# ucla-rlcourse/competitive-rl

Hardware: NVIDIA B200
Metric: cPongDouble env-steps/sec at 84x84x4 obs (higher is better)
Workload: dtype u8 obs / int32+f64 game state / f32 area-resize

## Files before the change

### competitive-rl_b200/csrc/crl_abi.cu

```cuda
#include <math.h>
#include <stdarg.h>
#include <stdio.h>
#include <stdlib.h>
#include <string.h>

#include <cuda.h>

#include <atomic>
#include <mutex>
#include <unordered_map>
#include <vector>

#include "../../include/crl_b200.h"
#include "crl_host.h"
#include "pong_common.cuh"

using namespace crl;

static thread_local char g_err[512] = "";
static std::atomic<uint64_t> g_launches{0};

static int fail(int code, const char* fmt, ...) {
    va_list ap;
    va_start(ap, fmt);
// ... 1 lines not shown
    va_end(ap);
    return code;
}

int crl_set_error(int code, const char* fmt, ...) {
    va_list ap;
    va_start(ap, fmt);
    vsnprintf(g_err, sizeof g_err, fmt, ap);
    va_end(ap);
    return code;
}
void crl_count_launch(int n) { g_launches += (uint64_t)n; }

#define CUDA_TRY(expr)                                                                                \
    do {                                                                                              \
        cudaError_t _e = (expr);                                                                      \
        if (_e != cudaSuccess) return fail(CRL_E_CUDA, "%s: %s", #expr, cudaGetErrorString(_e));      \
    } while (0)

#define LAUNCH(expr)     \
    do {                 \
        CUDA_TRY(expr);  \
        g_launches += 1; \
    } while (0)

struct crl_pong {
    crl_pong_config cfg;
    PongDev dev;
    std::vector<void*> allocs;
    double* serves_dev = nullptr;
    uint8_t* atlas_dev = nullptr;
    uint8_t* text_tab_dev = nullptr;
    uint8_t* tmpl_dev = nullptr;
    AreaTabs* tabs_dev = nullptr;
    AreaTabs tabs_host;
    uint8_t* fast_tabs_dev = nullptr;
    int32_t* actions_stage = nullptr;
    float* rew_stage = nullptr;
    uint8_t* done_stage = nullptr;
    int32_t* steps_stage = nullptr;
    float* real_stage = nullptr;
    bool atlas_loaded = false;
    bool was_reset = false;
    cudaStream_t copy_stream = nullptr;
    cudaEvent_t ev_state = nullptr, ev_copied = nullptr;
    struct ObsSet {
        uint8_t* obs[2];
        FrameSpec* shown;
        bool valid;
    };
    std::vector<ObsSet> sets;
    FrameSpec* shown_dev = nullptr;
    bool full_obs = false;
};

static size_t obs_bytes(const crl_pong* h) {
    return (size_t)h->dev.n * (h->dev.ring ? 2 * h->dev.c : h->dev.c) * h->dev.dim * h->dev.dim;
}

static void obs_written(crl_pong* h, const void* p, size_t bytes) {
    if (!p) return;
    const uintptr_t a = (uintptr_t)p, b = a + bytes, ob = obs_bytes(h);
    for (auto& st : h->sets)
        for (int k = 0; k < h->dev.n_agents; ++k)
            if (a < (uintptr_t)st.obs[k] + ob && (uintptr_t)st.obs[k] < b) st.valid = false;
}

static bool build_axis(int ssize, int dsize, uint8_t* src0, uint8_t* cnt, float (*alpha)[MAX_TAPS], uint8_t* first,
                       uint8_t* last) {
    const double scale = (double)ssize / dsize;
    for (int s = 0; s < ssize; ++s) { first[s] = 255; last[s] = 0; }
    for (int dx = 0; dx < dsize; ++dx) {
        const double fsx1 = dx * scale, fsx2 = fsx1 + scale;
        const double cell = fmin(scale, ssize - fsx1);
        int sx1 = (int)ceil(fsx1), sx2 = (int)floor(fsx2);
        sx2 = sx2 < ssize - 1 ? sx2 : ssize - 1;
        sx1 = sx1 < sx2 ? sx1 : sx2;
        int n = 0, s0 = -1;
        auto emit = [&](int s, float a) -> bool {
            if (n == 0) s0 = s;
            if (n >= MAX_TAPS || s != s0 + n) return false;
            alpha[dx][n++] = a;
            if (first[s] == 255) first[s] = (uint8_t)dx;
            last[s] = (uint8_t)dx;
            return true;
        };
        if (sx1 - fsx1 > 1e-3 && !emit(sx1 - 1, (float)((sx1 - fsx1) / cell))) return false;
        for (int sx = sx1; sx < sx2; ++sx)
            if (!emit(sx, (float)(1.0 / cell))) return false;
        if (fsx2 - sx2 > 1e-3 && !emit(sx2, (float)(fmin(fmin(fsx2 - sx2, 1.0), cell) / cell))) return false;
        if (n == 0) return false;
        src0[dx] = (uint8_t)s0;
        cnt[dx] = (uint8_t)n;
        for (int k = n; k < MAX_TAPS; ++k) alpha[dx][k] = 0.f;
    }
    for (int s = 0; s < ssize; ++s)
        if (first[s] == 255) return false;
    return true;
}

static bool build_tabs(int dim, AreaTabs* t) {
    memset(t, 0, sizeof *t);
    t->dim = dim;
    if (!build_axis(SCREEN_W, dim, t->x_src0, t->x_n, t->x_a, t->x_first, t->x_last)) return false;
    if (!build_axis(SCREEN_H, dim, t->y_src0, t->y_n, t->y_b, t->y_first, t->y_last)) return false;
    for (int dx = 0; dx < dim; ++dx)
// ... 62 lines not shown
    h->cfg = *cfg;
    PongDev& d = h->dev;
    memset(&d, 0, sizeof d);
    const size_t n = (size_t)cfg->num_envs;
    d.n = cfg->num_envs;
    d.n_agents = cfg->n_agents;
    d.dim = cfg->resized_dim;
    d.c = cfg->frame_stack > 0 ? cfg->frame_stack : 1;
    d.max_rounds = cfg->max_num_rounds;
    d.ring = cfg->stack_mode == 1 ? 1 : 0;
    d.zero_on_done = cfg->zero_on_done ? 1 : 0;
    d.first_env = cfg->first_env;
    d.seed = cfg->seed;
    const int dd = d.dim * d.dim;
    d.text_stride = ((tabs.text_rows * d.dim + 15) / 16) * 16;
    if (d.text_stride > ((dd + 15) / 16) * 16) d.text_stride = ((dd + 15) / 16) * 16;
    d.text_w0 = 0; d.text_w1 = d.text_stride / 4;
#define ALLOC(ptr, count)                                                        \
    do {                                                                         \
        cudaError_t _e = dev_alloc(h, &(ptr), (count));                          \
        if (_e != cudaSuccess) {                                                 \
            crl_pong_destroy(h);                                                 \
            return fail(CRL_E_CUDA, "cudaMalloc: %s", cudaGetErrorString(_e));   \
        }                                                                        \
    } while (0)
    ALLOC(d.ball, n); ALLOC(d.vx, n); ALLOC(d.vy, n); ALLOC(d.bats, n); ALLOC(d.score, n);
    ALLOC(d.num_steps, n); ALLOC(d.clip_steps, n); ALLOC(d.serve_count, n); ALLOC(d.last_done, n);
    ALLOC(d.skipbuf, 2 * n); ALLOC(d.hist, d.c * n); ALLOC(d.term_hist, d.c * n);
    ALLOC(d.serve_overrun, 1);
    ALLOC(d.stats, 8);
    ALLOC(d.work_counter, 2);
    ALLOC(h->tabs_dev, 1);
    ALLOC(h->atlas_dev, (size_t)CRL_PONG_ATLAS_BYTES);
    ALLOC(h->text_tab_dev, (size_t)ATLAS_SCORES * ATLAS_SCORES * 3 * 2 * d.text_stride);
    ALLOC(h->tmpl_dev, (size_t)((dd + 15) / 16) * 16);
    ALLOC(h->actions_stage, 2 * n); ALLOC(h->rew_stage, 2 * n); ALLOC(h->done_stage, n);
    ALLOC(h->steps_stage, n); ALLOC(h->real_stage, 2 * n);
    h->tabs_host = tabs;
    const size_t ftb = pong_fast_tabs_bytes(d.dim);
    if (ftb) {
        std::vector<uint8_t> img(ftb);
        if (pong_fast_tabs_fill(tabs, d.text_stride, img.data())) {
            ALLOC(h->fast_tabs_dev, ftb);
            cudaError_t _e = cudaMemcpy(h->fast_tabs_dev, img.data(), ftb, cudaMemcpyHostToDevice);
            if (_e == cudaSuccess) _e = launch_pong_build_bat_lut(d.dim, h->fast_tabs_dev, 0);
            if (_e != cudaSuccess) {
                crl_pong_destroy(h);
                return fail(CRL_E_CUDA, "fast tabs upload: %s", cudaGetErrorString(_e));
            }
            g_launches += 1;
            d.fast_tabs = h->fast_tabs_dev;
            d.quad_ok = (pong_quad_ok(tabs) && getenv("CRL_PONG_NO_QUAD") == nullptr) ? 1 : 0;
            h->full_obs = getenv("CRL_PONG_FULL_OBS") != nullptr;
        }
    }
    d.tabs = h->tabs_dev;
    d.atlas = h->atlas_dev;
    d.text_tab = h->text_tab_dev;
    d.tmpl = h->tmpl_dev;
#undef ALLOC
    e = cudaMemcpy(h->tabs_dev, &tabs, sizeof tabs, cudaMemcpyHostToDevice);
    if (e == cudaSuccess) e = pong_raster_init(d.raster_grid);
    if (e == cudaSuccess) e = launch_pong_construct(d, 0);
    if (e == cudaSuccess) e = cudaDeviceSynchronize();
    if (e != cudaSuccess) {
        crl_pong_destroy(h);
        return fail(CRL_E_CUDA, "construct: %s", cudaGetErrorString(e));
    }
    g_launches += 1;
    *out = h;
    return CRL_OK;
}

#define CHECK_HANDLE(h)                                        \
    do {                                                       \
        if (!(h)) return fail(CRL_E_INVALID, "null handle");   \
    } while (0);                                               \
    CrlDeviceGuard crl_guard_((h)->cfg.device);                \
    CUDA_TRY(crl_guard_.err)

int crl_pong_load_atlas(crl_pong* h, const uint8_t* strips_host, size_t bytes, void* stream) {
    CHECK_HANDLE(h);
    if (!strips_host || bytes != (size_t)CRL_PONG_ATLAS_BYTES)
        return fail(CRL_E_INVALID, "atlas must be %d bytes ([22][22][34][160][3] uint8)", CRL_PONG_ATLAS_BYTES);
    cudaStream_t s = (cudaStream_t)stream;
    {
        const AreaTabs& t = h->tabs_host;
        const int first = t.y_src0[t.text_rows - 1];
        bool white = true;
        for (int pair = 0; pair < ATLAS_SCORES * ATLAS_SCORES && white; ++pair)
            for (int r = first; r < ATLAS_ROWS && white; ++r) {
                const uint8_t* row = strips_host + ((size_t)pair * ATLAS_ROWS + r) * SCREEN_W * 3;
                for (int i = 0; i < SCREEN_W * 3; ++i)
                    if (row[i] != 255) { white = false; break; }
            }
        h->dev.fast_ok = white ? 1 : 0;
    }
    CUDA_TRY(cudaMemcpyAsync(h->atlas_dev, strips_host, bytes, cudaMemcpyHostToDevice, s));
    LAUNCH(launch_pong_build_tables(h->dev, h->text_tab_dev, h->tmpl_dev, s));
    CUDA_TRY(cudaStreamSynchronize(s));
    {
        const int tw = h->dev.text_stride / 4;
        const size_t n_ent = (size_t)ATLAS_SCORES * ATLAS_SCORES * 3 * 2;
        std::vector<uint32_t> tt(n_ent * tw), tm(tw);
        CUDA_TRY(cudaMemcpy(tt.data(), h->text_tab_dev, tt.size() * sizeof(uint32_t), cudaMemcpyDeviceToHost));
        CUDA_TRY(cudaMemcpy(tm.data(), h->tmpl_dev, tm.size() * sizeof(uint32_t), cudaMemcpyDeviceToHost));
        int w0 = tw, w1 = 0;
        for (int w = 0; w < tw; ++w) {
            bool differs = tm[w] != tt[w];
            for (size_t e = 1; e < n_ent && !differs; ++e) differs = tt[e * tw + w] != tt[w];
            if (differs) { if (w < w0) w0 = w; w1 = w + 1; }
        }
        if (w1 <= w0) w0 = w1 = 0;
        if (getenv("CRL_PONG_TEXT_FULL") != nullptr) { w0 = 0; w1 = tw; }
        h->dev.text_w0 = w0; h->dev.text_w1 = w1;
    }
    h->atlas_loaded = true;
    for (auto& st : h->sets) st.valid = false;
    return CRL_OK;
}

int crl_pong_inject_serves(crl_pong* h, const double* serves_host, int32_t k, void* stream) {
    CHECK_HANDLE(h);
    if (!serves_host || k < 3) return fail(CRL_E_INVALID, "serve table needs k >= 3 entries per env");
    cudaStream_t s = (cudaStream_t)stream;
    double* buf = nullptr;
    CUDA_TRY(dev_alloc(h, &buf, (size_t)h->dev.n * k * 2));
    CUDA_TRY(cudaMemcpyAsync(buf, serves_host, (size_t)h->dev.n * k * 2 * sizeof(double), cudaMemcpyHostToDevice, s));
    h->serves_dev = buf;
    h->dev.serves = buf;
    h->dev.serves_k = k;
    LAUNCH(launch_pong_construct(h->dev, s));
    CUDA_TRY(cudaStreamSynchronize(s));
    h->was_reset = false;
    return CRL_OK;
}

int crl_pong_seed(crl_pong* h, uint64_t seed) {
    CHECK_HANDLE(h);
    h->dev.seed = seed;
    return CRL_OK;
}

static int need_ready(crl_pong* h, bool need_reset) {
    if (!h->atlas_loaded) return fail(CRL_E_STATE, "crl_pong_load_atlas must be called before reset/step");
    if (need_reset && !h->was_reset) return fail(CRL_E_STATE, "reset must be called before step");
    return CRL_OK;
}

int crl_pong_render_obs(crl_pong* h, uint8_t* obs0_dev, uint8_t* obs1_dev, void* stream) {
    CHECK_HANDLE(h);
    if (int r = need_ready(h, true)) return r;
// ... 1 lines not shown
    if (h->dev.n_agents == 1) obs1_dev = obs0_dev;
    cudaStream_t s = (cudaStream_t)stream;
    crl_pong::ObsSet* set = nullptr;
    for (auto& st : h->sets)
        if (st.obs[0] == obs0_dev && (h->dev.n_agents == 1 || st.obs[1] == obs1_dev)) set = &st;
    const bool incremental = !h->full_obs && pong_raster_incremental_ok(h->dev, obs0_dev, obs1_dev);
    if (set && set->valid && incremental) {
        LAUNCH(launch_pong_raster(h->dev, h->dev.hist, obs0_dev, obs1_dev, set->shown, s));
        return CRL_OK;
    }
    LAUNCH(launch_pong_raster(h->dev, h->dev.hist, obs0_dev, obs1_dev, nullptr, s));
    if (!set) {
        obs_written(h, obs0_dev, obs_bytes(h));
        obs_written(h, obs1_dev, obs_bytes(h));
    } else if (incremental) {
        const size_t per_agent = (size_t)h->dev.c * h->dev.n;
        for (int k = 0; k < h->dev.n_agents; ++k)
            CUDA_TRY(cudaMemcpyAsync(set->shown + k * per_agent, h->dev.hist, per_agent * sizeof(FrameSpec),
                                     cudaMemcpyDeviceToDevice, s));
        set->valid = true;
    } else {
        set->valid = false;
    }
    return CRL_OK;
}

int crl_pong_set_obs_buffers(crl_pong* h, uint8_t* const* obs0_devs_host, uint8_t* const* obs1_devs_host, int32_t count,
                             void* stream) {
    CHECK_HANDLE(h);
    const int na = h->dev.n_agents;
    if (count != 0) {
        if (h->dev.ring) return fail(CRL_E_STATE, "stack_mode ring keeps its own frames: there are no buffer sets to register");
        if (count < 0 || count > CRL_PONG_MAX_OBS_SETS || !obs0_devs_host || (na == 2 && !obs1_devs_host))
            return fail(CRL_E_INVALID, "need 1 .. %d buffer sets (and obs1 buffers for cPongDouble), got %d",
                        CRL_PONG_MAX_OBS_SETS, count);
        std::vector<uint8_t*> all;
        for (int i = 0; i < count; ++i)
            for (int k = 0; k < na; ++k) {
                uint8_t* b = k ? obs1_devs_host[i] : obs0_devs_host[i];
                if (!b) return fail(CRL_E_INVALID, "null buffer in set %d", i);
                for (uint8_t* o : all)
                    if (o == b) return fail(CRL_E_INVALID, "a buffer appears twice in the sets");
                all.push_back(b);
            }
    }
    CUDA_TRY(cudaStreamSynchronize((cudaStream_t)stream));
    h->sets.clear();
    if (h->shown_dev) {
        CUDA_TRY(cudaFree(h->shown_dev));
        h->shown_dev = nullptr;
    }
    if (count == 0) return CRL_OK;
    const size_t per_set = (size_t)na * h->dev.c * h->dev.n;
    CUDA_TRY(cudaMalloc(&h->shown_dev, (size_t)count * per_set * sizeof(FrameSpec)));
    for (int i = 0; i < count; ++i)
        h->sets.push_back({{obs0_devs_host[i], na == 2 ? obs1_devs_host[i] : obs0_devs_host[i]}, h->shown_dev + i * per_set, false});
    return CRL_OK;
}

int crl_pong_forget_obs(crl_pong* h) {
    if (!h) return fail(CRL_E_INVALID, "null handle");
    for (auto& st : h->sets) st.valid = false;
    return CRL_OK;
}

int crl_pong_render_obs_generic(crl_pong* h, uint8_t* obs0_dev, uint8_t* obs1_dev, void* stream) {
    CHECK_HANDLE(h);
    if (int r = need_ready(h, true)) return r;
    if (!obs0_dev || (h->dev.n_agents == 2 && !obs1_dev)) return fail(CRL_E_INVALID, "null observation buffer");
    LAUNCH(launch_pong_raster_generic(h->dev, h->dev.hist, nullptr, h->dev.ring, obs0_dev, obs1_dev, (cudaStream_t)stream));
    obs_written(h, obs0_dev, obs_bytes(h));
    obs_written(h, obs1_dev, obs_bytes(h));
    return CRL_OK;
}

int crl_pong_render_obs_f32(crl_pong* h, int32_t terminal, const uint8_t* only_done_dev, float* obs0_dev, float* obs1_dev, void* stream) {
    CHECK_HANDLE(h);
    if (int r = need_ready(h, true)) return r;
    if (h->dev.ring) return fail(CRL_E_STATE, "float32 observations are plain stacks: create the handle with stack_mode 0");
    if (!obs0_dev || (h->dev.n_agents == 2 && !obs1_dev)) return fail(CRL_E_INVALID, "null observation buffer");
    LAUNCH(launch_pong_raster_f32(h->dev, terminal ? h->dev.term_hist : h->dev.hist, only_done_dev, obs0_dev, obs1_dev, (cudaStream_t)stream));
    obs_written(h, obs0_dev, 4 * obs_bytes(h));
    obs_written(h, obs1_dev, 4 * obs_bytes(h));
    return CRL_OK;
}

int crl_pong_reset_state(crl_pong* h, void* stream) {
    CHECK_HANDLE(h);
    if (int r = need_ready(h, false)) return r;
    LAUNCH(launch_pong_reset(h->dev, (cudaStream_t)stream));
    h->was_reset = true;
    h->dev.ring_phase = 0;
    h->dev.fill_all = 1;
    return CRL_OK;
}

int crl_pong_reset(crl_pong* h, uint8_t* obs0_dev, uint8_t* obs1_dev, void* stream) {
    CHECK_HANDLE(h);
    if (int r = need_ready(h, false)) return r;
    LAUNCH(launch_pong_reset(h->dev, (cudaStream_t)stream));
    h->was_reset = true;
    h->dev.ring_phase = 0;
    h->dev.fill_all = 1;
    return crl_pong_render_obs(h, obs0_dev, obs1_dev, stream);
}

// ... 255 lines not shown
```

### competitive-rl_b200/csrc/pong_common.cuh

```cuda
#pragma once
#include <cuda_runtime.h>
#include <stdint.h>

namespace crl {

constexpr int SCREEN_W = 160;
constexpr int SCREEN_H = 210;
constexpr int ARENA_TOP = 34;
constexpr int ARENA_BOTTOM = 194;
constexpr int ARENA_CENTERY = 114;
constexpr int BALL_SIZE = 4;
constexpr int BALL_X0 = 78;
constexpr int BALL_Y0 = 112;
constexpr int BAT_W = 5;
constexpr int BAT_H = 15;
constexpr int BAT_Y0 = 107;
constexpr int LEFT_BAT_X = 16;
constexpr int RIGHT_BAT_X = 139;
constexpr int SPEED = 4;
constexpr int MAX_STEP_PER_ROUND = 10000;
constexpr int CHEAT_CODES = 999;
constexpr int MIRROR_ROW = 25;
constexpr int ATLAS_ROWS = 34;
constexpr int ATLAS_SCORES = 22;
// ... 13 lines not shown
}

struct AreaTabs {
    int dim;
    int text_rows;
    uint8_t x_src0[MAX_DIM], x_n[MAX_DIM];
    uint8_t y_src0[MAX_DIM], y_n[MAX_DIM];
    float x_a[MAX_DIM][MAX_TAPS];
    float x_pa[MAX_DIM][MAX_TAPS];
    float y_b[MAX_DIM][MAX_TAPS];
    uint8_t x_first[SCREEN_W], x_last[SCREEN_W];
    uint8_t y_first[SCREEN_H], y_last[SCREEN_H];
};

struct PongDev {
    int n;
    int n_agents;
    int dim;
    int c;
    int max_rounds;
    int ring;
    int ring_phase;
    int fill_all;
    int zero_on_done;
    int64_t first_env;
    uint64_t seed;
    int32_t* ball;
    double* vx;
    double* vy;
    int32_t* bats;
    int32_t* score;
    int32_t* num_steps;
    int32_t* clip_steps;
    int32_t* serve_count;
    uint8_t* last_done;
    RenderState* skipbuf;
    FrameSpec* hist;
    FrameSpec* term_hist;
    const double* serves;
    int serves_k;
    int32_t* serve_overrun;
    unsigned long long* stats;
    unsigned long long* work_counter;
    const AreaTabs* tabs;
    const uint8_t* atlas;
    const uint8_t* text_tab;
    const uint8_t* tmpl;
    int text_stride;
    int text_w0, text_w1;
    const void* fast_tabs;
    int fast_ok;
    int raster_grid[3];
    int quad_ok;
};

__host__ __device__ inline void philox4x32_10(uint32_t c0, uint32_t c1, uint32_t c2, uint32_t c3, uint32_t k0,
                                              uint32_t k1, uint32_t out[4]) {
    for (int r = 0; r < 10; ++r) {
        uint64_t p0 = (uint64_t)0xD2511F53u * c0;
        uint64_t p1 = (uint64_t)0xCD9E8D57u * c2;
        uint32_t n0 = (uint32_t)(p1 >> 32) ^ c1 ^ k0;
        uint32_t n1 = (uint32_t)p1;
        uint32_t n2 = (uint32_t)(p0 >> 32) ^ c3 ^ k1;
        uint32_t n3 = (uint32_t)p0;
        c0 = n0; c1 = n1; c2 = n2; c3 = n3;
        k0 += 0x9E3779B9u;
        k1 += 0xBB67AE85u;
    }
    out[0] = c0; out[1] = c1; out[2] = c2; out[3] = c3;
}

cudaError_t launch_pong_construct(const PongDev& p, cudaStream_t s);
cudaError_t launch_pong_reset(const PongDev& p, cudaStream_t s);
cudaError_t launch_pong_step(const PongDev& p, const int32_t* actions, float* rew, uint8_t* done, int32_t* num_steps,
                             float* real_reward, cudaStream_t s);
cudaError_t launch_pong_get_state(const PongDev& p, double* state, cudaStream_t s);
cudaError_t launch_pong_set_state(const PongDev& p, const double* state, cudaStream_t s);
cudaError_t launch_pong_random_actions(int32_t* actions, int n_values, uint64_t seed, uint64_t step, cudaStream_t s);

cudaError_t launch_pong_build_tables(const PongDev& p, uint8_t* text_tab, uint8_t* tmpl, cudaStream_t s);
cudaError_t launch_pong_raster(const PongDev& p, const FrameSpec* hist, uint8_t* obs0, uint8_t* obs1, FrameSpec* shown,
                               cudaStream_t s);
bool pong_raster_incremental_ok(const PongDev& p, const void* obs0, const void* obs1);
cudaError_t launch_pong_raster_generic(const PongDev& p, const FrameSpec* hist, const uint8_t* only_done, int ring,
                                       uint8_t* obs0, uint8_t* obs1, cudaStream_t s);
cudaError_t launch_pong_raster_f32(const PongDev& p, const FrameSpec* hist, const uint8_t* only_done, float* obs0, float* obs1,
                                   cudaStream_t s);
cudaError_t pong_raster_init(int grid_out[3]);
bool pong_quad_ok(const AreaTabs& a);
size_t pong_fast_tabs_bytes(int dim);
bool pong_fast_tabs_fill(const AreaTabs& a, int text_stride, void* host_buf);
cudaError_t launch_pong_build_bat_lut(int dim, void* fast_tabs_dev, cudaStream_t s);
cudaError_t launch_pong_raw_frame(const PongDev& p, int env, uint8_t* rgb0, uint8_t* rgb1, cudaStream_t s);

}
```

### competitive-rl_b200/csrc/pong_raster_fast.cu

```cuda
#include <type_traits>

#include "pong_raster_dev.cuh"

namespace crl {

template <int TAPS> struct alignas(16) TapEnt;
template <> struct alignas(16) TapEnt<3> { uint32_t meta; float w[3]; };
template <> struct alignas(16) TapEnt<5> { uint32_t meta; float w[5]; uint32_t pad[2]; };

#ifndef CRL_FAST84_CTAS
#define CRL_FAST84_CTAS 3
#endif
template <int DIM> struct FastCfg;
template <> struct FastCfg<84> { static constexpr int TAPS = 3, VEC = 16, CTAS = CRL_FAST84_CTAS; };
template <> struct FastCfg<42> { static constexpr int TAPS = 5, VEC = 4, CTAS = 3; };

constexpr int FAST_WARPS = 8;
constexpr int FIRST_PAD = 224;
constexpr int BAT_ROWS = 8;

template <int DIM> struct alignas(16) FastTabs {
    TapEnt<FastCfg<DIM>::TAPS> xe[DIM], ye[DIM];
    uint32_t bat_lut[2][DIM][1 << FastCfg<DIM>::TAPS];
    float xlut[DIM][1 << FastCfg<DIM>::TAPS];
// ... 133 lines not shown
    any_valid = va || vb;
    if (!va) f.y = f.w;
    if (!vb) f.w = f.y;
    const int pairA = (int)(f.y & 255u) * ATLAS_SCORES + (int)((f.y >> 8) & 255u);
    const int pairB = (int)(f.w & 255u) * ATLAS_SCORES + (int)((f.w >> 8) & 255u);
    int base = pairA, kind = 0;
    if (pairA != pairB) {
        const int d = pairB - pairA;
        if (d == ATLAS_SCORES) kind = 1;
        else if (d == 1 && (pairA % ATLAS_SCORES) != ATLAS_SCORES - 1) kind = 2;
        else if (d == -ATLAS_SCORES) { base = pairB; kind = 1; }
        else if (d == -1 && (pairB % ATLAS_SCORES) != ATLAS_SCORES - 1) { base = pairB; kind = 2; }
        else return -2;
    }
    return (base * 3 + kind) * 2 + agent;
}

template <int DIM>
__device__ __forceinline__ void frame_patch_offsets(const FastTabs<DIM>* T, FrameSpec f, int agent, int lane, int& bat_off,
                                                    int& ball_off) {
    const int cL = (int)T->bat_c0[0], cR = (int)T->bat_c0[1];
    const int b_side = lane >> 4, b_which = (lane >> 3) & 1, b_row = lane & 7;
    const int p_which = lane >> 4, p_col = lane & 3, p_row = (lane >> 2) & 3;
    if (!((f.y >> 16) & 1u)) { f.x = f.z; f.y = f.w; }
    if (!((f.w >> 16) & 1u)) { f.z = f.x; f.w = f.y; }
    const bool same = (f.x == f.z);
    const int lyA = (f.x >> 16) & 255u, ryA = f.x >> 24, lyB = (f.z >> 16) & 255u, ryB = f.z >> 24;
    const int vlA = agent ? ryA : lyA, vrA = agent ? lyA : ryA;
    const int vlB = agent ? ryB : lyB, vrB = agent ? lyB : ryB;
    bat_off = -1;
    {
        const int y0 = b_which ? (b_side ? vrB : vlB) : (b_side ? vrA : vlA);
        const int c0 = max(y0, ARENA_TOP), c1 = min(y0 + BAT_H, ARENA_BOTTOM);
        if (c1 > c0 && !(b_which && same)) {
            const int dy = (int)T->y_first[c0] + b_row;
            if (dy <= (int)T->y_last[c1 - 1]) bat_off = dy * DIM + (b_side ? cR : cL);
        }
    }
    ball_off = -1;
    {
        const FrameSpec& g = f;
        const uint32_t bx = p_which ? g.z : g.x;
        int x0 = bx & 255u, x1 = min(x0 + BALL_SIZE, SCREEN_W);
        int y0 = (bx >> 8) & 255u, y1 = min(y0 + BALL_SIZE, ARENA_BOTTOM);
        y0 = max(y0, ARENA_TOP);
        if (agent) { const int t = SCREEN_W - x1; x1 = SCREEN_W - x0; x0 = t; }
        if (x1 > x0 && y1 > y0 && !(p_which && same)) {
            const int dx = (int)T->x_first[x0] + p_col, dy = (int)T->y_first[y0] + p_row;
            if (dx <= (int)T->x_last[x1 - 1] && dy <= (int)T->y_last[y1 - 1]) ball_off = dy * DIM + dx;
        }
    }
}

template <int DIM, bool RING, bool INC>
__global__ void __launch_bounds__(FAST_WARPS * 32, FastCfg<DIM>::CTAS)
pong_raster_fast_kernel(PongDev p, const FrameSpec* __restrict__ hist, uint8_t* __restrict__ obs0,
                        uint8_t* __restrict__ obs1, const FastTabs<DIM>* __restrict__ gtabs, FrameSpec* __restrict__ shown) {
    constexpr int TAPS = FastCfg<DIM>::TAPS, VEC = FastCfg<DIM>::VEC;
    constexpr int DD = DIM * DIM, FB = ((DD + 15) / 16) * 16, NCH = DD / VEC;
#ifndef CRL_RASTER_TMA
#define CRL_RASTER_TMA 0
#endif
    constexpr bool USE_TMA = (DD % 16 == 0) && (CRL_RASTER_TMA != 0) && !INC;
    constexpr int TEXT_ITERS = 3;
    typedef typename VecT<VEC>::type V;
    typedef FastTabs<DIM> Tabs;
    static_assert(DD % VEC == 0, "frame must be a whole number of store vectors");
    static_assert(!INC || (!RING && VEC == 16), "incremental stacks: 16-byte chunks, plain stacks");

    extern __shared__ uint4 smem_raw[];
    uint8_t* smem = reinterpret_cast<uint8_t*>(smem_raw);
    const Tabs* T = reinterpret_cast<const Tabs*>(smem);
    const int lane = threadIdx.x & 31, warp = threadIdx.x >> 5;
    uint8_t* sm8 = smem + sizeof(Tabs) + (size_t)warp * FB;
    V* sm = reinterpret_cast<V*>(sm8);

    {
        const uint4* src = reinterpret_cast<const uint4*>(gtabs);
        uint4* dst = reinterpret_cast<uint4*>(smem);
        for (int i = threadIdx.x; i < (int)(sizeof(Tabs) / 16); i += blockDim.x) dst[i] = src[i];
        const uint4* tm = reinterpret_cast<const uint4*>(p.tmpl);
        uint4* f = reinterpret_cast<uint4*>(sm8);
        for (int i = lane; i < FB / 16; i += 32) f[i] = tm[i];
    }
    __syncthreads();

    const int text_chunks = p.text_stride / VEC;
    const int cL = (int)T->bat_c0[0], cR = (int)T->bat_c0[1];
    const int b_side = lane >> 4, b_which = (lane >> 3) & 1, b_row = lane & 7;
    const int p_which = lane >> 4, p_col = lane & 3, p_row = (lane >> 2) & 3;
    int prev_bat_off = -1, prev_ball_off = -1;
    uint32_t prev_bat_rest = 0u, prev_ball_old = 0u;
    int cur_text = -1;
    bool pending = false;
    FrameSpec prev_spec = make_uint4(0u, 0u, 0u, 0u);
    bool prev_known = false;

    const long long n_stacks = (long long)p.n * p.n_agents;
    const int per_ticket = INC ? CRL_INC_TICKET : max(1, 4 / (RING ? 2 : p.c));
    const int out_slots = RING ? 2 * p.c : p.c;
    long long s = 0, s_end = 0;
    for (;;) {
        if (s >= s_end) {
            unsigned long long ticket = 0ull;
            if (lane == 0) ticket = atomicAdd(p.work_counter, (unsigned long long)per_ticket);
            s = (long long)__shfl_sync(0xffffffffu, ticket, 0);
            s_end = min(s + per_ticket, n_stacks);
            if (s >= n_stacks) break;
        }
        const long long s_cur = s++;
        const int env = (int)(s_cur / p.n_agents), agent = (int)(s_cur % p.n_agents);
        uint8_t* out_stack = (agent ? obs1 : obs0) + (size_t)env * out_slots * DD;
        FrameSpec my_spec = make_uint4(0u, 0u, 0u, 0u), my_shown = make_uint4(0u, 0u, 0u, 0u);
        FrameSpec* shown_at = INC ? shown + ((size_t)agent * p.c + lane) * p.n + env : nullptr;
        if (lane < p.c) {
            my_spec = hist[(size_t)lane * p.n + env];
            if (INC) my_shown = *shown_at;
        }
        const int first_slot = (RING && !p.fill_all && !p.last_done[env]) ? p.c - 1 : 0;

        for (int slot = first_slot; slot < p.c; ++slot) {
            FrameSpec f;
            f.x = __shfl_sync(0xffffffffu, my_spec.x, slot);
            f.y = __shfl_sync(0xffffffffu, my_spec.y, slot);
            f.z = __shfl_sync(0xffffffffu, my_spec.z, slot);
            f.w = __shfl_sync(0xffffffffu, my_spec.w, slot);
            const FrameSpec f_raw = f;
            FrameSpec o = f;
            if (INC) {
                o.x = __shfl_sync(0xffffffffu, my_shown.x, slot);
                o.y = __shfl_sync(0xffffffffu, my_shown.y, slot);
                o.z = __shfl_sync(0xffffffffu, my_shown.z, slot);
                o.w = __shfl_sync(0xffffffffu, my_shown.w, slot);
                if (spec_diff(f, o) == 0u) continue;
            }
            uint8_t* out8 = out_stack + (size_t)slot * DD;
            uint8_t* out8b = nullptr;
            if (RING) {
                const int pos = p.ring_phase + 1 + slot;
                out8 = out_stack + (size_t)pos * DD;
                out8b = out_stack + (size_t)(pos >= p.c ? pos - p.c : pos + p.c) * DD;
            }

            const bool va = (f.y >> 16) & 1u, vb = (f.w >> 16) & 1u;
            if (!va) { f.x = f.z; f.y = f.w; }
            if (!vb) { f.z = f.x; f.w = f.y; }
            const int pairA = (int)(f.y & 255u) * ATLAS_SCORES + (int)((f.y >> 8) & 255u);
            const int pairB = (int)(f.w & 255u) * ATLAS_SCORES + (int)((f.w >> 8) & 255u);
            int base = pairA, kind = 0;
            bool text_ok = true;
            if (pairA != pairB) {
                const int d = pairB - pairA;
                if (d == ATLAS_SCORES) kind = 1;
                else if (d == 1 && (pairA % ATLAS_SCORES) != ATLAS_SCORES - 1) kind = 2;
                else if (d == -ATLAS_SCORES) { base = pairB; kind = 1; }
                else if (d == -1 && (pairB % ATLAS_SCORES) != ATLAS_SCORES - 1) { base = pairB; kind = 2; }
                else text_ok = false;
            }

            if (!(va || vb)) {
                V z;
                memset(&z, 0, sizeof z);
                V* out = reinterpret_cast<V*>(out8);
                for (int k = lane; k < NCH; k += 32) st_stream(out + k, z);
                if (RING) {
                    V* outb = reinterpret_cast<V*>(out8b);
                    for (int k = lane; k < NCH; k += 32) st_stream(outb + k, z);
                }
                continue;
            }

            const bool same = (f.x == f.z);
            const int lyA = (f.x >> 16) & 255u, ryA = f.x >> 24, lyB = (f.z >> 16) & 255u, ryB = f.z >> 24;
            const int vlA = agent ? ryA : lyA, vrA = agent ? lyA : ryA;
            const int vlB = agent ? ryB : lyB, vrB = agent ? lyB : ryB;

            const int text_id = text_ok ? (base * 3 + kind) * 2 + agent : -2;
            const bool reload_text = text_id != cur_text || !text_ok;
            const uint8_t* __restrict__ te8 = p.text_tab + (size_t)text_id * p.text_stride;
            if (reload_text && text_ok && lane * 128 < p.text_stride)
                asm volatile("prefetch.global.L1 [%0];" ::"l"(te8 + lane * 128));

            int bat_off = -1;
            uint32_t bat_val = 0u, bat_rest = 0u;
            {
                const int yA = b_side ? vrA : vlA, yB = b_side ? vrB : vlB;
                const int y0 = b_which ? yB : yA;
                const int c0 = max(y0, ARENA_TOP), c1 = min(y0 + BAT_H, ARENA_BOTTOM);
                if (c1 > c0 && !(b_which && same)) {
                    const int dy = (int)T->y_first[c0] + b_row;
                    if (dy <= (int)T->y_last[c1 - 1]) {
                        const uint32_t meta = T->ye[dy].meta;
                        const int sy0 = meta & 255u;
                        const int a0 = max(yA, ARENA_TOP), a1 = min(yA + BAT_H, ARENA_BOTTOM);
                        const int b0 = max(yB, ARENA_TOP), b1 = min(yB + BAT_H, ARENA_BOTTOM);
                        uint32_t vbits = 0u;
                        if (a1 > a0) vbits |= tap_bits(((1u << (a1 - a0)) - 1u) << 8, a0, sy0);
                        if (b1 > b0) vbits |= tap_bits(((1u << (b1 - b0)) - 1u) << 8, b0, sy0);
                        vbits &= (meta >> 8) & 255u;
                        bat_val = T->bat_lut[b_side][dy][vbits];
                        bat_rest = T->bat_lut[b_side][dy][0];
                        bat_off = dy * DIM + (b_side ? cR : cL);
                    }
                }
            }

            int ball_off = -1;
            uint32_t ball_val = 0u;
            {
                int ax0 = f.x & 255u, ax1 = min(ax0 + BALL_SIZE, SCREEN_W);
                int ay0 = (f.x >> 8) & 255u, ay1 = min(ay0 + BALL_SIZE, ARENA_BOTTOM);
                ay0 = max(ay0, ARENA_TOP);
                int bx0 = f.z & 255u, bx1 = min(bx0 + BALL_SIZE, SCREEN_W);
                int by0 = (f.z >> 8) & 255u, by1 = min(by0 + BALL_SIZE, ARENA_BOTTOM);
                by0 = max(by0, ARENA_TOP);
                if (agent) {
                    int t = SCREEN_W - ax1; ax1 = SCREEN_W - ax0; ax0 = t;
                    t = SCREEN_W - bx1; bx1 = SCREEN_W - bx0; bx0 = t;
                }
                const bool ea = ax1 > ax0 && ay1 > ay0, eb = bx1 > bx0 && by1 > by0 && !same;
                const int mx0 = p_which ? bx0 : ax0, mx1 = p_which ? bx1 : ax1;
                const int my0 = p_which ? by0 : ay0, my1 = p_which ? by1 : ay1;
                if (p_which ? eb : ea) {
                    const int dx = (int)T->x_first[mx0] + p_col, dy = (int)T->y_first[my0] + p_row;
                    if (dx <= (int)T->x_last[mx1 - 1] && dy <= (int)T->y_last[my1 - 1]) {
                        const TapEnt<TAPS> X = T->xe[dx], Y = T->ye[dy];
                        const int sx0 = X.meta & 255u, sy0 = Y.meta & 255u;
                        const uint32_t xmask = (X.meta >> 8) & 255u, ymask = (Y.meta >> 8) & 255u;
                        uint32_t pat = xmask * spread6((Y.meta >> 16) & 255u);
                        if (ea)
                            pat |= (tap_bits(((1u << (ax1 - ax0)) - 1u) << 8, ax0, sx0) & xmask) *
                                   spread6(tap_bits(((1u << (ay1 - ay0)) - 1u) << 8, ay0, sy0) & ymask);
                        if (eb)
                            pat |= (tap_bits(((1u << (bx1 - bx0)) - 1u) << 8, bx0, sx0) & xmask) *
                                   spread6(tap_bits(((1u << (by1 - by0)) - 1u) << 8, by0, sy0) & ymask);
                        const bool nl = (unsigned)(dx - cL) < 4u, nr = (unsigned)(dx - cR) < 4u;
                        if (nl || nr) {
                            const int yA = nr ? vrA : vlA, yB = nr ? vrB : vlB;
                            const int a0 = max(yA, ARENA_TOP), a1 = min(yA + BAT_H, ARENA_BOTTOM);
                            const int b0 = max(yB, ARENA_TOP), b1 = min(yB + BAT_H, ARENA_BOTTOM);
                            uint32_t vbits = 0u;
                            if (a1 > a0) vbits |= tap_bits(((1u << (a1 - a0)) - 1u) << 8, a0, sy0);
                            if (b1 > b0) vbits |= tap_bits(((1u << (b1 - b0)) - 1u) << 8, b0, sy0);
                            const uint32_t hb = tap_bits(((1u << BAT_W) - 1u) << 8, nr ? RIGHT_BAT_X : LEFT_BAT_X, sx0);
                            pat |= (hb & xmask) * spread6(vbits & ymask);
                        }
                        ball_val = eval_from_pat_lut<TAPS>(T->xlut[dx], Y, pat);
                        ball_off = dy * DIM + dx;
                    }
                }
            }

            bool whole = true;
            int ta = 0, tb = 0, old_bat = -1, old_ball = -1;
            if (INC) {
                bool old_valid;
                const int old_text = frame_text_id(o, agent, old_valid);
                whole = !old_valid || old_text == -2 || !text_ok;
                if (!whole && old_text != text_id) { ta = p.text_w0 * 4 >> 4; tb = min((p.text_w1 * 4 + 15) >> 4, NCH); }
                if (!whole) {
                    if (prev_known && spec_diff(o, prev_spec) == 0u) { old_bat = prev_bat_off; old_ball = prev_ball_off; }
                    else frame_patch_offsets<DIM>(T, o, agent, lane, old_bat, old_ball);
                }
            }

            if (pending) {
                if (lane == 0) bulk_wait_read();
                __syncwarp();
            }
            if (prev_bat_off >= 0) {
                if (DIM % 4 == 0) {
                    *reinterpret_cast<uint32_t*>(sm8 + prev_bat_off) = prev_bat_rest;
                } else {
#pragma unroll
                    for (int j = 0; j < 4; ++j) sm8[prev_bat_off + j] = (uint8_t)(prev_bat_rest >> (8 * j));
                }
            }
            __syncwarp();
            if (prev_ball_off >= 0) sm8[prev_ball_off] = (uint8_t)prev_ball_old;
            __syncwarp();
            if (reload_text) {
                if (text_ok) {
                    const V* __restrict__ te = reinterpret_cast<const V*>(te8);
#pragma unroll
                    for (int j = 0; j < TEXT_ITERS; ++j)
                        if (lane + 32 * j < text_chunks) sm[lane + 32 * j] = te[lane + 32 * j];
                } else {
                    const int n_text = p.tabs->text_rows * DIM;
                    for (int i = lane; i < n_text; i += 32)
                        sm8[i] = eval_text_pixel(p.tabs, p.atlas, pairA, pairB, agent != 0, i / DIM, i % DIM);
                }
                cur_text = text_id;
                __syncwarp();
            }
            uint32_t ball_old = 0u;
            if (ball_off >= 0) ball_old = sm8[ball_off];
            __syncwarp();
            if (bat_off >= 0) {
                if (DIM % 4 == 0) {
                    *reinterpret_cast<uint32_t*>(sm8 + bat_off) = bat_val;
                } else {
#pragma unroll
                    for (int j = 0; j < 4; ++j) sm8[bat_off + j] = (uint8_t)(bat_val >> (8 * j));
                }
            }
            __syncwarp();
            if (ball_off >= 0) sm8[ball_off] = (uint8_t)ball_val;
            prev_bat_off = bat_off; prev_bat_rest = bat_rest;
            prev_ball_off = ball_off; prev_ball_old = ball_old;
            prev_spec = f_raw; prev_known = true;

#ifdef CRL_RASTER_NO_DRAIN
            continue;
#endif
// ... 399 lines not shown
        const int y1 = y + BALL_SIZE < ARENA_BOTTOM ? y + BALL_SIZE : ARENA_BOTTOM;
        if (a.y_last[y1 - 1] - a.y_first[y] + 1 > 2) return false;
    }
    return true;
}

bool pong_quad_ok(const AreaTabs& a) { return a.dim == 42 && quad_geometry_ok<42>(a); }

template <int DIM>
static size_t quad_smem_bytes() {
    return sizeof(QuadTabs<DIM>) + (size_t)QUAD_WARPS * 4 * DIM * DIM;
}

template <int DIM>
static size_t fast_smem_bytes() {
    constexpr int FB = ((DIM * DIM + 15) / 16) * 16;
    return sizeof(FastTabs<DIM>) + (size_t)FAST_WARPS * FB;
}

size_t pong_fast_tabs_bytes(int dim) {
    return dim == 84 ? sizeof(FastTabs<84>) : dim == 42 ? sizeof(FastTabs<42>) : 0;
}

bool pong_fast_tabs_fill(const AreaTabs& a, int text_stride, void* host_buf) {
    if (a.dim == 84) return text_stride <= 96 * 16 && fill_fast_tabs<84>(a, reinterpret_cast<FastTabs<84>*>(host_buf));
    if (a.dim == 42) return text_stride <= 96 * 4 && fill_fast_tabs<42>(a, reinterpret_cast<FastTabs<42>*>(host_buf));
    return false;
}

cudaError_t launch_pong_build_bat_lut(int dim, void* fast_tabs_dev, cudaStream_t s) {
    if (dim == 84) {
        pong_build_bat_lut_kernel<84><<<(2 * 84 * 8 + 127) / 128, 128, 0, s>>>(reinterpret_cast<FastTabs<84>*>(fast_tabs_dev));
        pong_build_xlut_kernel<84><<<(84 * 8 + 127) / 128, 128, 0, s>>>(reinterpret_cast<FastTabs<84>*>(fast_tabs_dev));
    } else if (dim == 42) {
        pong_build_bat_lut_kernel<42><<<(2 * 42 * 32 + 127) / 128, 128, 0, s>>>(reinterpret_cast<FastTabs<42>*>(fast_tabs_dev));
        pong_build_xlut_kernel<42><<<(42 * 32 + 127) / 128, 128, 0, s>>>(reinterpret_cast<FastTabs<42>*>(fast_tabs_dev));
    }
    return cudaGetLastError();
}

cudaError_t pong_raster_init(int g_grid[3]) {
    cudaError_t e;
    int dev = 0, sms = 0, nb = 0;
    if ((e = cudaGetDevice(&dev)) != cudaSuccess) return e;
    if ((e = cudaDeviceGetAttribute(&sms, cudaDevAttrMultiProcessorCount, dev)) != cudaSuccess) return e;
    const void* fast[2][2] = {{(const void*)pong_raster_fast_kernel<84, false, false>, (const void*)pong_raster_fast_kernel<84, true, false>},
                              {(const void*)pong_raster_fast_kernel<42, false, false>, (const void*)pong_raster_fast_kernel<42, true, false>}};
    const int smem[2] = {(int)fast_smem_bytes<84>(), (int)fast_smem_bytes<42>()};
    for (int d = 0; d < 2; ++d)
        for (int r = 0; r < 2; ++r)
            if ((e = cudaFuncSetAttribute(fast[d][r], cudaFuncAttributeMaxDynamicSharedMemorySize, smem[d])) != cudaSuccess) return e;
    e = cudaFuncSetAttribute(pong_raster_fast_kernel<84, false, true>, cudaFuncAttributeMaxDynamicSharedMemorySize, smem[0]);
    if (e != cudaSuccess) return e;
    e = cudaOccupancyMaxActiveBlocksPerMultiprocessor(&nb, pong_raster_fast_kernel<84, false, false>, FAST_WARPS * 32, smem[0]);
    if (e != cudaSuccess) return e;
    g_grid[0] = sms * max(min(nb, FastCfg<84>::CTAS), 1);
    e = cudaOccupancyMaxActiveBlocksPerMultiprocessor(&nb, pong_raster_fast_kernel<42, false, false>, FAST_WARPS * 32, smem[1]);
    if (e != cudaSuccess) return e;
    g_grid[1] = sms * max(nb, 1);
    e = cudaFuncSetAttribute(pong_raster_quad_kernel<42>, cudaFuncAttributeMaxDynamicSharedMemorySize, (int)quad_smem_bytes<42>());
    if (e != cudaSuccess) return e;
    e = cudaOccupancyMaxActiveBlocksPerMultiprocessor(&nb, pong_raster_quad_kernel<42>, QUAD_WARPS * 32, quad_smem_bytes<42>());
    if (e != cudaSuccess) return e;
    g_grid[2] = sms * max(nb, 1);
    return cudaSuccess;
}

static bool fast_path(const PongDev& p, const void* obs0, const void* obs1) {
    const bool aligned = ((uintptr_t)obs0 % 16 == 0) && ((uintptr_t)obs1 % 16 == 0);
    return p.fast_tabs != nullptr && p.fast_ok && aligned && (p.dim == 84 || p.dim == 42);
}

bool pong_raster_incremental_ok(const PongDev& p, const void* obs0, const void* obs1) {
    return fast_path(p, obs0, obs1) && p.dim == 84 && !p.ring;
}

cudaError_t launch_pong_raster(const PongDev& p, const FrameSpec* hist, uint8_t* obs0, uint8_t* obs1, FrameSpec* shown,
                               cudaStream_t s) {
    const long long n_stacks = (long long)p.n * p.n_agents;
    if (n_stacks == 0) return cudaSuccess;
    if (shown && !pong_raster_incremental_ok(p, obs0, obs1)) return cudaErrorInvalidValue;
    if (!fast_path(p, obs0, obs1)) return launch_pong_raster_generic(p, hist, nullptr, p.ring, obs0, obs1, s);
    const long long want = (n_stacks + FAST_WARPS - 1) / FAST_WARPS;
    cudaError_t me = cudaMemsetAsync(p.work_counter, 0, sizeof(unsigned long long), s);
    if (me != cudaSuccess) return me;
    if (p.dim == 84) {
        const unsigned grid = (unsigned)min((long long)p.raster_grid[0], want);
        const FastTabs<84>* tabs = reinterpret_cast<const FastTabs<84>*>(p.fast_tabs);
        if (shown) {
            pong_raster_fast_kernel<84, false, true><<<grid, FAST_WARPS * 32, fast_smem_bytes<84>(), s>>>(p, hist, obs0, obs1, tabs, shown);
        } else if (p.ring) {
            pong_raster_fast_kernel<84, true, false><<<grid, FAST_WARPS * 32, fast_smem_bytes<84>(), s>>>(p, hist, obs0, obs1, tabs, nullptr);
        } else {
            pong_raster_fast_kernel<84, false, false><<<grid, FAST_WARPS * 32, fast_smem_bytes<84>(), s>>>(p, hist, obs0, obs1, tabs, nullptr);
        }
    } else if (p.quad_ok && !p.ring && (long long)p.n * p.c * p.n_agents < (1LL << 31)) {
        const long long quads = (((long long)p.n * p.c + 3) / 4) * p.n_agents;
        const unsigned grid = (unsigned)min((long long)p.raster_grid[2], (quads + 4 * QUAD_WARPS - 1) / (4 * QUAD_WARPS));
        pong_raster_quad_kernel<42><<<grid, QUAD_WARPS * 32, quad_smem_bytes<42>(), s>>>(
            p, hist, obs0, obs1, reinterpret_cast<const FastTabs<42>*>(p.fast_tabs));
    } else {
        const unsigned grid = (unsigned)min((long long)p.raster_grid[1], want);
        const FastTabs<42>* tabs = reinterpret_cast<const FastTabs<42>*>(p.fast_tabs);
        if (p.ring) pong_raster_fast_kernel<42, true, false><<<grid, FAST_WARPS * 32, fast_smem_bytes<42>(), s>>>(p, hist, obs0, obs1, tabs, nullptr);
        else pong_raster_fast_kernel<42, false, false><<<grid, FAST_WARPS * 32, fast_smem_bytes<42>(), s>>>(p, hist, obs0, obs1, tabs, nullptr);
    }
    return cudaGetLastError();
}

}
```

Measured before the change: 162.3 million.

## Cache per-frame bat/ball patch records to skip recomputing area-resize patches

Adds a per-env, per-agent cache of compact patch records (bat row offset, vbits, ball offset and value) tagged by frame spec. The incremental 84x84 raster kernel reuses them instead of re-evaluating the bat and ball resize patches and old-frame offsets. Records are written into free slots when a frame is newly rendered. This cuts the arithmetic and table lookups per frame in exchange for extra global loads and stores, a warp ballot, and higher register pressure.

```diff
diff --git a/competitive-rl_b200/csrc/crl_abi.cu b/competitive-rl_b200/csrc/crl_abi.cu
--- a/competitive-rl_b200/csrc/crl_abi.cu
+++ b/competitive-rl_b200/csrc/crl_abi.cu
@@ -77,6 +77,7 @@
     std::vector<ObsSet> sets;
     FrameSpec* shown_dev = nullptr;
     bool full_obs = false;
+    bool patch_cache = false;
 };
 
 static size_t obs_bytes(const crl_pong* h) {
@@ -245,6 +246,8 @@
             d.fast_tabs = h->fast_tabs_dev;
             d.quad_ok = (pong_quad_ok(tabs) && getenv("CRL_PONG_NO_QUAD") == nullptr) ? 1 : 0;
             h->full_obs = getenv("CRL_PONG_FULL_OBS") != nullptr;
+            h->patch_cache = d.dim == 84 && !d.ring && d.c <= PATCH_CACHE_MAX_STACK &&
+                             getenv("CRL_PONG_NO_PATCH_CACHE") == nullptr;
         }
     }
     d.tabs = h->tabs_dev;
@@ -291,6 +294,8 @@
     }
     CUDA_TRY(cudaMemcpyAsync(h->atlas_dev, strips_host, bytes, cudaMemcpyHostToDevice, s));
     LAUNCH(launch_pong_build_tables(h->dev, h->text_tab_dev, h->tmpl_dev, s));
+    if (h->dev.rec_tag)
+        CUDA_TRY(cudaMemsetAsync(h->dev.rec_tag, 0, (size_t)h->dev.n_agents * h->dev.c * h->dev.n * sizeof(FrameSpec), s));
     CUDA_TRY(cudaStreamSynchronize(s));
     {
         const int tw = h->dev.text_stride / 4;
@@ -398,6 +403,10 @@
     }
     if (count == 0) return CRL_OK;
     const size_t per_set = (size_t)na * h->dev.c * h->dev.n;
+    if (h->patch_cache && !h->dev.rec) {
+        CUDA_TRY(dev_alloc(h, &h->dev.rec_tag, per_set));
+        CUDA_TRY(dev_alloc(h, &h->dev.rec, per_set * 32));
+    }
     CUDA_TRY(cudaMalloc(&h->shown_dev, (size_t)count * per_set * sizeof(FrameSpec)));
     for (int i = 0; i < count; ++i)
         h->sets.push_back({{obs0_devs_host[i], na == 2 ? obs1_devs_host[i] : obs0_devs_host[i]}, h->shown_dev + i * per_set, false});
diff --git a/competitive-rl_b200/csrc/pong_common.cuh b/competitive-rl_b200/csrc/pong_common.cuh
--- a/competitive-rl_b200/csrc/pong_common.cuh
+++ b/competitive-rl_b200/csrc/pong_common.cuh
@@ -89,7 +89,11 @@
     int fast_ok;
     int raster_grid[3];
     int quad_ok;
+    FrameSpec* rec_tag;
+    uint32_t* rec;
 };
+
+constexpr int PATCH_CACHE_MAX_STACK = 4;
 
 __host__ __device__ inline void philox4x32_10(uint32_t c0, uint32_t c1, uint32_t c2, uint32_t c3, uint32_t k0,
                                               uint32_t k1, uint32_t out[4]) {
diff --git a/competitive-rl_b200/csrc/pong_raster_fast.cu b/competitive-rl_b200/csrc/pong_raster_fast.cu
--- a/competitive-rl_b200/csrc/pong_raster_fast.cu
+++ b/competitive-rl_b200/csrc/pong_raster_fast.cu
@@ -209,7 +209,19 @@
     }
 }
 
-template <int DIM, bool RING, bool INC>
+template <int DIM>
+__device__ __forceinline__ void rec_patch_offsets(uint32_t r, int bat_col, int& bat_off, int& ball_off) {
+    bat_off = (r & 127u) ? ((int)(r & 127u) - 1) * DIM + bat_col : -1;
+    ball_off = (int)((r >> 10) & 8191u) - 1;
+}
+
+__device__ __forceinline__ uint32_t rec_pick(const uint32_t (&w)[PATCH_CACHE_MAX_STACK], uint32_t hit) {
+    static_assert(PATCH_CACHE_MAX_STACK == 4, "one select per entry");
+    const int e = (__ffs(hit) - 1) >> 2;
+    return e == 0 ? w[0] : e == 1 ? w[1] : e == 2 ? w[2] : w[3];
+}
+
+template <int DIM, bool RING, bool INC, bool CACHE = false>
 __global__ void __launch_bounds__(FAST_WARPS * 32, FastCfg<DIM>::CTAS)
 pong_raster_fast_kernel(PongDev p, const FrameSpec* __restrict__ hist, uint8_t* __restrict__ obs0,
                         uint8_t* __restrict__ obs1, const FastTabs<DIM>* __restrict__ gtabs, FrameSpec* __restrict__ shown) {
@@ -224,6 +236,7 @@
     typedef FastTabs<DIM> Tabs;
     static_assert(DD % VEC == 0, "frame must be a whole number of store vectors");
     static_assert(!INC || (!RING && VEC == 16), "incremental stacks: 16-byte chunks, plain stacks");
+    static_assert(!CACHE || (INC && TAPS == 3 && DD < 8191), "patch records: incremental stacks, 3-bit tap sets, 13-bit offsets");
 
     extern __shared__ uint4 smem_raw[];
     uint8_t* smem = reinterpret_cast<uint8_t*>(smem_raw);
@@ -270,7 +283,22 @@
         uint8_t* out_stack = (agent ? obs1 : obs0) + (size_t)env * out_slots * DD;
         FrameSpec my_spec = make_uint4(0u, 0u, 0u, 0u), my_shown = make_uint4(0u, 0u, 0u, 0u);
         FrameSpec* shown_at = INC ? shown + ((size_t)agent * p.c + lane) * p.n + env : nullptr;
-        if (lane < p.c) {
+        uint32_t match = 0u, free_e = 0u, rec_w[PATCH_CACHE_MAX_STACK];
+        uint32_t* rec_at = nullptr;
+        if (CACHE) {
+            const int q_k = lane & 3, q_e = (lane >> 2) & 3;
+            FrameSpec q_tag = make_uint4(0u, 0u, 0u, 0u);
+            if (q_k < p.c) my_spec = (lane >> 4) ? shown[((size_t)agent * p.c + q_k) * p.n + env] : hist[(size_t)q_k * p.n + env];
+            if (q_e < p.c) q_tag = p.rec_tag[((size_t)agent * p.c + q_e) * p.n + env];
+            rec_at = p.rec + ((size_t)agent * p.n + env) * p.c * 32 + lane;
+#pragma unroll
+            for (int e = 0; e < PATCH_CACHE_MAX_STACK; ++e) rec_w[e] = e < p.c ? rec_at[e * 32] : 0u;
+            const bool tag_valid = ((q_tag.y | q_tag.w) >> 16) & 1u;
+            match = __ballot_sync(0xffffffffu, q_k < p.c && q_e < p.c && tag_valid && spec_diff(my_spec, q_tag) == 0u);
+#pragma unroll
+            for (int e = 0; e < PATCH_CACHE_MAX_STACK; ++e)
+                if (e < p.c && ((match >> (4 * e)) & 15u) == 0u) free_e |= 1u << e;
+        } else if (lane < p.c) {
             my_spec = hist[(size_t)lane * p.n + env];
             if (INC) my_shown = *shown_at;
         }
@@ -284,7 +312,13 @@
             f.w = __shfl_sync(0xffffffffu, my_spec.w, slot);
             const FrameSpec f_raw = f;
             FrameSpec o = f;
-            if (INC) {
+            if (CACHE) {
+                o.x = __shfl_sync(0xffffffffu, my_spec.x, 16 + slot);
+                o.y = __shfl_sync(0xffffffffu, my_spec.y, 16 + slot);
+                o.z = __shfl_sync(0xffffffffu, my_spec.z, 16 + slot);
+                o.w = __shfl_sync(0xffffffffu, my_spec.w, 16 + slot);
+                if (spec_diff(f, o) == 0u) continue;
+            } else if (INC) {
                 o.x = __shfl_sync(0xffffffffu, my_shown.x, slot);
                 o.y = __shfl_sync(0xffffffffu, my_shown.y, slot);
                 o.z = __shfl_sync(0xffffffffu, my_shown.z, slot);
@@ -338,8 +372,20 @@
             if (reload_text && text_ok && lane * 128 < p.text_stride)
                 asm volatile("prefetch.global.L1 [%0];" ::"l"(te8 + lane * 128));
 
-            int bat_off = -1;
-            uint32_t bat_val = 0u, bat_rest = 0u;
+            int bat_off = -1, ball_off = -1;
+            uint32_t bat_val = 0u, bat_rest = 0u, ball_val = 0u;
+            const uint32_t hit = CACHE ? (match >> slot) & 0x1111u : 0u;
+            if (CACHE && hit) {
+                const uint32_t r = rec_pick(rec_w, hit);
+                rec_patch_offsets<DIM>(r, b_side ? cR : cL, bat_off, ball_off);
+                if (bat_off >= 0) {
+                    const int dy = (int)(r & 127u) - 1;
+                    bat_val = T->bat_lut[b_side][dy][(r >> 7) & 7u];
+                    bat_rest = T->bat_lut[b_side][dy][0];
+                }
+                ball_val = r >> 23;
+            } else {
+            uint32_t rec_word = 0u;
             {
                 const int yA = b_side ? vrA : vlA, yB = b_side ? vrB : vlB;
                 const int y0 = b_which ? yB : yA;
@@ -358,12 +404,11 @@
                         bat_val = T->bat_lut[b_side][dy][vbits];
                         bat_rest = T->bat_lut[b_side][dy][0];
                         bat_off = dy * DIM + (b_side ? cR : cL);
+                        if (CACHE) rec_word = (uint32_t)(dy + 1) | vbits << 7;
                     }
                 }
             }
 
-            int ball_off = -1;
-            uint32_t ball_val = 0u;
             {
                 int ax0 = f.x & 255u, ax1 = min(ax0 + BALL_SIZE, SCREEN_W);
                 int ay0 = (f.x >> 8) & 255u, ay1 = min(ay0 + BALL_SIZE, ARENA_BOTTOM);
@@ -404,8 +449,17 @@
                         }
                         ball_val = eval_from_pat_lut<TAPS>(T->xlut[dx], Y, pat);
                         ball_off = dy * DIM + dx;
+                        if (CACHE) rec_word |= (uint32_t)(ball_off + 1) << 10 | ball_val << 23;
                     }
                 }
+            }
+
+            if (CACHE && text_ok && free_e != 0u && !(prev_known && spec_diff(f_raw, prev_spec) == 0u)) {
+                const int e = __ffs(free_e) - 1;
+                free_e &= free_e - 1u;
+                rec_at[e * 32] = rec_word;
+                if (lane == 0) p.rec_tag[((size_t)agent * p.c + e) * p.n + env] = f_raw;
+            }
             }
 
             bool whole = true;
@@ -416,7 +470,9 @@
                 whole = !old_valid || old_text == -2 || !text_ok;
                 if (!whole && old_text != text_id) { ta = p.text_w0 * 4 >> 4; tb = min((p.text_w1 * 4 + 15) >> 4, NCH); }
                 if (!whole) {
+                    const uint32_t old_hit = CACHE ? (match >> (16 + slot)) & 0x1111u : 0u;
                     if (prev_known && spec_diff(o, prev_spec) == 0u) { old_bat = prev_bat_off; old_ball = prev_ball_off; }
+                    else if (CACHE && old_hit) rec_patch_offsets<DIM>(rec_pick(rec_w, old_hit), b_side ? cR : cL, old_bat, old_ball);
                     else frame_patch_offsets<DIM>(T, o, agent, lane, old_bat, old_ball);
                 }
             }
@@ -922,6 +978,8 @@
             if ((e = cudaFuncSetAttribute(fast[d][r], cudaFuncAttributeMaxDynamicSharedMemorySize, smem[d])) != cudaSuccess) return e;
     e = cudaFuncSetAttribute(pong_raster_fast_kernel<84, false, true>, cudaFuncAttributeMaxDynamicSharedMemorySize, smem[0]);
     if (e != cudaSuccess) return e;
+    e = cudaFuncSetAttribute(pong_raster_fast_kernel<84, false, true, true>, cudaFuncAttributeMaxDynamicSharedMemorySize, smem[0]);
+    if (e != cudaSuccess) return e;
     e = cudaOccupancyMaxActiveBlocksPerMultiprocessor(&nb, pong_raster_fast_kernel<84, false, false>, FAST_WARPS * 32, smem[0]);
     if (e != cudaSuccess) return e;
     g_grid[0] = sms * max(min(nb, FastCfg<84>::CTAS), 1);
@@ -957,7 +1015,9 @@
     if (p.dim == 84) {
         const unsigned grid = (unsigned)min((long long)p.raster_grid[0], want);
         const FastTabs<84>* tabs = reinterpret_cast<const FastTabs<84>*>(p.fast_tabs);
-        if (shown) {
+        if (shown && p.rec && p.c <= PATCH_CACHE_MAX_STACK) {
+            pong_raster_fast_kernel<84, false, true, true><<<grid, FAST_WARPS * 32, fast_smem_bytes<84>(), s>>>(p, hist, obs0, obs1, tabs, shown);
+        } else if (shown) {
             pong_raster_fast_kernel<84, false, true><<<grid, FAST_WARPS * 32, fast_smem_bytes<84>(), s>>>(p, hist, obs0, obs1, tabs, shown);
         } else if (p.ring) {
             pong_raster_fast_kernel<84, true, false><<<grid, FAST_WARPS * 32, fast_smem_bytes<84>(), s>>>(p, hist, obs0, obs1, tabs, nullptr);
```

After: 163.1 million (median of 6 runs). No clear change (+0.5%).
